# NLAFET/SpLLT

Hardware: AMD Instinct MI355X
Metric: factorize GFLOP/s (fp64) (higher is better)
Workload: dtype f64; 1 GPU; nd24k_like; stand_in_for=SuiteSparse ND/nd24k, n=72324, nnz_lower=10970712, nb=256, nnz_L=190279977, nnodes=684, ordering=user/geometric-nd, parallelism=1 GPU, level-batched stream DAG (chain / bulk / far streams, zone pipeline)

## Files before the change

spllt_amd/csrc/kernels.hip:

```cpp
#include <hip/hip_runtime.h>

#include <cstdint>
#include <cstdlib>
#include <tuple>
#include <type_traits>

#include "kernels.hpp"

#ifndef UPD128_BK
#define UPD128_BK 16
#endif
#ifndef UPD128_WM
#define UPD128_WM 4
#define UPD128_WN 2
#endif

#ifndef UPD64_OCC
#define UPD64_OCC 0
#endif

#if defined(SCATTER_EXPERIMENT) && SCATTER_EXPERIMENT == 1
#define SCATTER_ADD(p, v) (*(p) += (v))
#elif defined(SCATTER_EXPERIMENT) && SCATTER_EXPERIMENT == 2
#define SCATTER_ADD(p, v) (*(p) = (v))
// ... 202 lines not shown
          if (failcol == (1 << 30)) failcol = j;
          djj = 1.0;
        }
        double y, d;
        rsqrt_sqrt(djj, y, d);
        const double sc = row[j] * (y * y);
        wx[j] = (((lr == j) ? 1.0 : 0.0) - wacc[j]) * y;
        const double z = wx[j] * y;
#pragma unroll
        for (int k = j + 1; k < 16; ++k) {
          row[k] -= sc * tk[k];
          wacc[k] = __builtin_fma(tk[k], z, wacc[k]);
        }
        row[j] = (lr == j) ? d : row[j] * y;
        RI[J * 16 + j] = y;
        asm volatile("" : "+v"(wx[j]));
      }
      if (lane < 16) {
#pragma unroll
        for (int c = 0; c < 16; ++c) {
          T[(J * 16 + lr) * TLD + J * 16 + c] = (c <= lr) ? row[c] : 0.0;
          DI[J][c * DLD + lr] = wx[c];
          X[(J * 16 + c) * TLD + J * 16 + lr] = wx[c];
        }
        if (failcol != (1 << 30) && lane == 0 && !(u.flags & 4)) atomicMin(flag, u.gcol + J * 16 + failcol + 1);
      }
    }
    __syncthreads();
    STAMP(3 + 3 * J);
    {
      const int I = J + 1 + w;
      if (I < nblk) {
        d4 acc = {0.0, 0.0, 0.0, 0.0};
#pragma unroll
        for (int t = 0; t < 4; ++t) {
          const double a = T[(I * 16 + lr) * TLD + J * 16 + 4 * t + lq];
          const double b = DI[J][lr * DLD + 4 * t + lq];
          acc = __builtin_amdgcn_mfma_f64_16x16x4f64(a, b, acc, 0, 0, 0);
        }
        st_c(T, I * 16, J * 16, lane, acc);
      }
    }
    __syncthreads();
    STAMP(4 + 3 * J);
  }
  if (!do_chol && w < nblk) {
    double x[16];
#pragma unroll
    for (int i = 0; i < 16; ++i) {
      double sacc = (i == lr) ? 1.0 : 0.0;
#pragma unroll
      for (int k = 0; k < i; ++k) sacc -= T[(w * 16 + i) * TLD + w * 16 + k] * x[k];
      x[i] = (i >= lr) ? sacc * RI[w * 16 + i] : 0.0;
    }
    if (lane < 16) {
#pragma unroll
      for (int i = 0; i < 16; ++i) {
        DI[w][i * DLD + lr] = x[i];
        X[(w * 16 + i) * TLD + w * 16 + lr] = x[i];
      }
    }
  }
  __syncthreads();
  STAMP(14);
  for (int d = 1; d < nblk; ++d) {
    const int J = w, I = J + d;
    if (I < nblk) {
      d4 S = {0.0, 0.0, 0.0, 0.0};
      for (int K = J; K < I; ++K) {
#pragma unroll
        for (int k = 0; k < 16; k += 4) {
          const double a = T[(I * 16 + lr) * TLD + K * 16 + k + lq];
          const double b = X[(K * 16 + k + lq) * TLD + J * 16 + lr];
          S = __builtin_amdgcn_mfma_f64_16x16x4f64(a, b, S, 0, 0, 0);
        }
      }
      d4 R = {0.0, 0.0, 0.0, 0.0};
#pragma unroll
      for (int t = 0; t < 4; ++t) {
        const double a = -DI[I][lr * DLD + 4 * t + lq];
        R = __builtin_amdgcn_mfma_f64_16x16x4f64(a, S[t], R, 0, 0, 0);
      }
      st_c(X, I * 16, J * 16, lane, R);
    }
    __syncthreads();
  }
  STAMP(15);
  if (tid < 256 && lc < n) {
    const bool st_l = do_chol && !(u.flags & 2), st_i = !(u.flags & 4);
#pragma unroll
    for (int e = 0; e < 16; ++e) {
      const int r = 4 * e + lw;
      if (r < n) {
        if (st_l && lc <= r) A[(int64_t)r * ld + lc] = T[r * TLD + lc];
        if (st_i) D[(int64_t)r * ldd + lc] = X[r * TLD + lc];
      }
    }
  }
  STAMP(16);
  (void)np;
}

template <int B, int E, class F>
__device__ __forceinline__ void static_for(F&& f) {
  if constexpr (B < E) {
    f(std::integral_constant<int, B>{});
    static_for<B + 1, E>(f);
  }
}
template <int K>
__device__ __forceinline__ void fmac_bc(double& acc, double s0, double s1) {
  asm volatile("v_fmac_f64_dpp %0, %1, %2 row_newbcast:%3 row_mask:0xf bank_mask:0xf" : "+v"(acc) : "v"(s0), "v"(s1), "n"(K));
}
template <int K>
__device__ __forceinline__ void fmac_bc_pivot(double& acc, double s0, double s1, double& d) {
  asm volatile("v_fmac_f64_dpp %0, %2, %3 row_newbcast:%4 row_mask:0xf bank_mask:0xf\n\ts_nop 1\n\t"
               "v_mov_b64_dpp %1, %0 row_newbcast:%4 row_mask:0xf bank_mask:0xf"
               : "+v"(acc), "=&v"(d) : "v"(s0), "v"(s1), "n"(K));
}
__device__ __forceinline__ double rcp_newton(double d) {
  double y = __builtin_amdgcn_rcp(d);
  y = __builtin_fma(y, __builtin_fma(-d, y, 1.0), y);
  y = __builtin_fma(y, __builtin_fma(-d, y, 1.0), y);
  return y;
}
__device__ __forceinline__ double a_rcp(double d) {
  double y;
  asm volatile("v_rcp_f64 %0, %1\n\ts_nop 0" : "=v"(y) : "v"(d));
  return y;
}
__device__ __forceinline__ double a_nr_err(double d, double y) {
  double e;
  asm volatile("v_fma_f64 %0, -%1, %2, 1.0" : "=v"(e) : "v"(d), "v"(y));
  return e;
}
__device__ __forceinline__ void a_nr_fix(double& y, double e) {
  asm volatile("v_fma_f64 %0, %0, %1, %0" : "+v"(y) : "v"(e));
}
__device__ __forceinline__ double a_nmul(double a, double b) {
  double o;
  asm volatile("v_mul_f64 %0, %1, -%2" : "=v"(o) : "v"(a), "v"(b));
  return o;
}
__device__ __forceinline__ double a_mul(double a, double b) {
  double o;
  asm volatile("v_mul_f64 %0, %1, %2" : "=v"(o) : "v"(a), "v"(b));
  return o;
}
__device__ __forceinline__ double a_sub(double a, double b) {
  double o;
  asm volatile("v_add_f64 %0, %1, -%2" : "=v"(o) : "v"(a), "v"(b));
  return o;
}
__device__ __forceinline__ int chol16_regs(double (&row)[16], double (&wx)[16], int lr) {
  double wacc[16], delta[16];
#pragma unroll
  for (int c = 0; c < 16; ++c) {
    wacc[c] = 0.0;
    delta[c] = (lr == c) ? 1.0 : 0.0;
  }
  double dn = bcast_row<0>(row[0]);
  double dmine = dn;
  double y = rcp_newton(dn);
  STAMP2(true, 21);
  static_for<0, 16>([&](auto jc) {
    constexpr int j = decltype(jc)::value;
    using std::integral_constant;
    const double nsc = a_nmul(row[j], y);
    if constexpr (j + 1 < 16) {
      constexpr int nR = 14 - j, nF = 29 - 2 * j;
      double wxj = 0.0, z = 0.0;
      auto fill = [&](auto lo, auto hi) {
        static_for<decltype(lo)::value, decltype(hi)::value>([&](auto ic) {
          constexpr int i = decltype(ic)::value;
          if constexpr (i < nR) {
            fmac_bc<j + 2 + i>(row[j + 2 + i], row[j], nsc);
          } else {
            if constexpr (i == nR) {
              wxj = a_sub(delta[j], wacc[j]);
              z = a_mul(wxj, y);
            }
            fmac_bc<j + 1 + i - nR>(wacc[j + 1 + i - nR], row[j], z);
          }
        });
      };
      constexpr int b0 = nF * 30 / 100, b1 = nF * 44 / 100, b2 = nF * 58 / 100, b3 = nF * 72 / 100;
      fmac_bc_pivot<j + 1>(row[j + 1], row[j], nsc, dn);
      double yn = a_rcp(dn);
      fill(integral_constant<int, 0>{}, integral_constant<int, b0>{});
      double e = a_nr_err(dn, yn);
      fill(integral_constant<int, b0>{}, integral_constant<int, b1>{});
      a_nr_fix(yn, e);
      fill(integral_constant<int, b1>{}, integral_constant<int, b2>{});
      e = a_nr_err(dn, yn);
      fill(integral_constant<int, b2>{}, integral_constant<int, b3>{});
      a_nr_fix(yn, e);
      fill(integral_constant<int, b3>{}, integral_constant<int, nF>{});
      dmine = (lr == j + 1) ? dn : dmine;
      wx[j] = wxj;
      y = yn;
    } else {
      wx[j] = delta[j] - wacc[j];
    }
  });
  STAMP2(true, 22);
  double ys, rs;
  rsqrt_sqrt(dmine, ys, rs);
  static_for<0, 16>([&](auto cc) {
    constexpr int c = decltype(cc)::value;
    const double sc = bcast_row<c>(ys);
    row[c] *= sc;
    wx[c] *= sc;
    asm volatile("" : "+v"(row[c]), "+v"(wx[c]));
  });
  (void)rs;
  STAMP2(true, 23);
  const unsigned long long bad = __ballot(!(dmine > 0.0)) & 0xffffull;
  return bad ? __builtin_ctzll(bad) : (1 << 30);
}

__device__ __forceinline__ void potrf64_v2(PotrfShared& sh, double* __restrict__ A, int ld, int n,
                                           double* __restrict__ D, int ldd, int gcol, int flags,
                                           int* __restrict__ flag) {
  double (&T)[64 * TLD] = sh.T;
  double (&X)[64 * TLD] = sh.X;
  const int tid = threadIdx.x;
  const int lane = tid & 63, w = tid >> 6, lq = lane >> 4, lr = lane & 15;
  const int nblk = (n + 15) >> 4;
  const bool st_l = !(flags & 2), st_i = !(flags & 4), x_lower = (flags & 8) != 0;
  STAMP(0);
  const int lw = tid >> 6, lc = tid & 63;
  if (flags & 16) {
    if (tid < 256) {
#pragma unroll
      for (int e = 0; e < 16; ++e) X[(4 * e + lw) * TLD + lc] = 0.0;
    }
  } else
  if (tid < 256) {
    double v[16];
#pragma unroll
    for (int e = 0; e < 16; ++e) {
      const int r = 4 * e + lw;
      const int cmax = min(n - 1, r | 15);
      v[e] = A[(int64_t)(r < n ? r : n - 1) * ld + (lc < cmax ? lc : cmax)];
    }
#pragma unroll
    for (int e = 0; e < 16; ++e) X[(4 * e + lw) * TLD + lc] = 0.0;
#pragma unroll
    for (int e = 0; e < 16; ++e) {
      const int r = 4 * e + lw;
      T[r * TLD + lc] = (r < n && lc <= r) ? v[e] : ((r == lc) ? 1.0 : 0.0);
    }
  }
  __syncthreads();
  STAMP(1);
  auto store_rows8 = [&](double* __restrict__ dst, int ldst, const double* M, int row0, int col0) {
    const int g = row0 + (lane >> 3), c = col0 + 2 * (lane & 7);
    const int cend = min(g, n - 1);
    if (g >= n || c > cend) return;
    const double v0 = M[g * TLD + c], v1 = M[g * TLD + c + 1];
    double* q = dst + (int64_t)g * ldst + c;
    if (c + 1 <= cend) {
      typedef double d2 __attribute__((ext_vector_type(2), aligned(8)));
      *reinterpret_cast<d2*>(q) = (d2){v0, v1};
    } else {
      q[0] = v0;
    }
  };
  auto upd_block = [&](int I, int Jp, int S) {
    d4 acc = ld_c(T, I * 16, Jp * 16, lane);
    double a[4], b[4];
#pragma unroll
    for (int t = 0; t < 4; ++t) {
      a[t] = -T[(I * 16 + lr) * TLD + S * 16 + 4 * t + lq];
      b[t] = T[(Jp * 16 + lr) * TLD + S * 16 + 4 * t + lq];
    }
#pragma unroll
    for (int t = 0; t < 4; ++t) acc = __builtin_amdgcn_mfma_f64_16x16x4f64(a[t], b[t], acc, 0, 0, 0);
    st_c(T, I * 16, Jp * 16, lane, acc);
  };
  d4 Xpre = {0.0, 0.0, 0.0, 0.0};
  auto shadow = [&](int S, int ws, int ns, bool stores) {
    const int K = ws;
    if (K < S) {
      d4 R = {0.0, 0.0, 0.0, 0.0};
#pragma unroll
      for (int tt = 0; tt < 4; ++tt) {
        const double a = -X[(S * 16 + lr) * TLD + S * 16 + 4 * tt + lq];
        R = __builtin_amdgcn_mfma_f64_16x16x4f64(a, Xpre[tt], R, 0, 0, 0);
      }
      st_c(X, S * 16, K * 16, lane, R);
      if (st_i && x_lower) {
#pragma unroll
        for (int r = 0; r < 4; ++r) {
          const int g = S * 16 + lq + 4 * r;
          if (g < n) D[(int64_t)g * ldd + K * 16 + lr] = R[r];
        }
      }
    }
    int t = 0;
    for (int Jp = S + 1; Jp < nblk; ++Jp)
      for (int I = Jp; I < nblk; ++I) {
        if (I == S + 1 && Jp == S + 1) continue;
        if (t++ % ns == ws) upd_block(I, Jp, S);
      }
    if (S + 1 < nblk && K <= S) {
      Xpre = (d4){0.0, 0.0, 0.0, 0.0};
      for (int M = K; M <= S; ++M) {
#pragma unroll
        for (int k = 0; k < 16; k += 4) {
          const double a = T[((S + 1) * 16 + lr) * TLD + M * 16 + k + lq];
          const double b = X[(M * 16 + k + lq) * TLD + K * 16 + lr];
          Xpre = __builtin_amdgcn_mfma_f64_16x16x4f64(a, b, Xpre, 0, 0, 0);
        }
      }
    }
    if (!stores) return;
    const int ngrp = (64 - S * 16) / 8;
    for (int gi = ws; gi < ngrp; gi += ns)
      if (st_l) store_rows8(A, ld, T, S * 16 + gi * 8, S * 16);
    if (st_i && x_lower)
      for (int gi = ws; gi < 2; gi += ns) store_rows8(D, ldd, X, S * 16 + gi * 8, S * 16);
  };
  for (int J = 0; J < nblk; ++J) {
    if (w == 0) {
      if (J > 0) upd_block(J, J, J - 1);
      double row[16], wx[16];
      STAMP2(true, 20);
#pragma unroll
      for (int c = 0; c < 16; ++c) row[c] = T[(J * 16 + lr) * TLD + J * 16 + c];
      const int failcol = chol16_regs(row, wx, lr);
      STAMP2(true, 24);
      if (lq == 0) {
        double* dst = &T[(J * 16 + lr) * TLD + J * 16];
#pragma unroll
        for (int c = 0; c < 16; ++c) dst[c] = row[c];
        if (failcol != (1 << 30) && lane == 0 && st_i) atomicMin(flag, gcol + J * 16 + failcol + 1);
      } else if (lq == 1) {
        double* dst = &X[(J * 16) * TLD + J * 16 + lr];
#pragma unroll
        for (int c = 0; c < 16; ++c) dst[c * TLD] = wx[c];
      }
      STAMP2(true, 25);
    } else if (w < 4 && J > 0) {
      shadow(J - 1, w - 1, 3, true);
    }
    __syncthreads();
    STAMP(2 + 2 * J);
    if (w < 4 && J + 1 + w < nblk) {
      const int I = J + 1 + w;
      d4 acc = {0.0, 0.0, 0.0, 0.0};
#pragma unroll
      for (int t = 0; t < 4; ++t) {
        const double a = T[(I * 16 + lr) * TLD + J * 16 + 4 * t + lq];
        const double b = X[(J * 16 + lr) * TLD + J * 16 + 4 * t + lq];
        acc = __builtin_amdgcn_mfma_f64_16x16x4f64(a, b, acc, 0, 0, 0);
      }
      st_c(T, I * 16, J * 16, lane, acc);
    }
    __syncthreads();
    STAMP(3 + 2 * J);
  }
  if (w > 0 && w < 4) {
    const int S = nblk - 1, K = w - 1;
    if (K < S) shadow(S, K, 3, false);
  } else if (w == 0) {
    const int S = nblk - 1;
    if (st_l) { store_rows8(A, ld, T, S * 16, S * 16); store_rows8(A, ld, T, S * 16 + 8, S * 16); }
    if (st_i && x_lower) { store_rows8(D, ldd, X, S * 16, S * 16); store_rows8(D, ldd, X, S * 16 + 8, S * 16); }
  }
  STAMP(10);
  if (st_i && !x_lower) {
    __syncthreads();
    if (tid < 256)
      for (int r = lw; r < n; r += 4)
        if (lc < n) D[(int64_t)r * ldd + lc] = X[r * TLD + lc];
  }
  STAMP(11);
}

__device__ __forceinline__ void potrf64(PotrfShared& sh, double* __restrict__ A, int ld, int n,
                                        double* __restrict__ D, int ldd, int gcol, int flags,
                                        int* __restrict__ flag) {
#ifndef POTRF_V1
  if (!(flags & 1)) {
    potrf64_v2(sh, A, ld, n, D, ldd, gcol, flags, flag);
    return;
  }
#endif
  potrf64_body(sh, A, ld, n, D, ldd, gcol, flags, flag);
}

__global__ __launch_bounds__(256) void k_potrf_panel(const PotrfUnit* __restrict__ units,
                                                     double* __restrict__ L,
                                                     double* __restrict__ dinv,
                                                     int* __restrict__ flag, const PotrfUnit u0) {
  __shared__ PotrfShared sh;
  __builtin_amdgcn_s_setprio(3);
  const PotrfUnit u = blockIdx.x == 0 ? u0 : units[blockIdx.x];
  potrf64(sh, L + u.off, u.ld, u.n, dinv + u.dinv_off, u.n, u.gcol, u.flags, flag);
}

__global__ __launch_bounds__(256) void k_chain_potrf(const ChainUnit* __restrict__ units,
                                                     double* __restrict__ L,
                                                     double* __restrict__ dinv,
                                                     int* __restrict__ flag, const ChainUnit u0) {
  __shared__ PotrfShared sh;
  __builtin_amdgcn_s_setprio(3);
  const ChainUnit u = blockIdx.x == 0 ? u0 : units[blockIdx.x];
  const int cq = u.c0 - u.cs;
  potrf64(sh, L + u.off + (int64_t)u.c0 * u.ld + u.c0, u.ld, u.pn, dinv + u.winv_off + cq, u.ce - u.cs,
          u.gcol, 8, flag);
}

constexpr int kPanelThreads = 512;

__device__ __forceinline__ void stage_block(double* __restrict__ dst, const double* __restrict__ src,
                                            int64_t ld, int nrow, int ncol, int tid) {
  const int r = tid >> 3, cl = tid & 7;
  const double* row = src + (int64_t)(r < nrow ? r : nrow - 1) * ld;
  double v[8];
#pragma unroll
  for (int e = 0; e < 8; ++e) v[e] = row[cl + 8 * e < ncol ? cl + 8 * e : ncol - 1];
#pragma unroll
  for (int e = 0; e < 8; ++e) dst[r * TLD + cl + 8 * e] = (r < nrow && cl + 8 * e < ncol) ? v[e] : 0.0;
}

__device__ __forceinline__ void mma_64(const double* __restrict__ a, const double* __restrict__ b, int s,
                                       int jb0, int lane, d4& acc0, d4& acc1) {
  const int lq = lane >> 4, lr = lane & 15;
  double av[16], b0[16], b1[16];
#pragma unroll
  for (int kt = 0; kt < 16; ++kt) {
    av[kt] = a[(s * 16 + lr) * TLD + 4 * kt + lq];
    b0[kt] = b[(jb0 * 16 + lr) * TLD + 4 * kt + lq];
    b1[kt] = b[((jb0 + 1) * 16 + lr) * TLD + 4 * kt + lq];
  }
#pragma unroll
  for (int kt = 0; kt < 16; ++kt) {
    acc0 = __builtin_amdgcn_mfma_f64_16x16x4f64(av[kt], b0[kt], acc0, 0, 0, 0);
    acc1 = __builtin_amdgcn_mfma_f64_16x16x4f64(av[kt], b1[kt], acc1, 0, 0, 0);
  }
}

__device__ __forceinline__ void mma_64_lean(const double* __restrict__ a, const double* __restrict__ b, int s,
                                            int jb0, int lane, d4& acc0, d4& acc1) {
  const int lq = lane >> 4, lr = lane & 15;
#pragma unroll
  for (int hf = 0; hf < 2; ++hf) {
    double av[8], b0[8], b1[8];
#pragma unroll
    for (int kt = 0; kt < 8; ++kt) {
      av[kt] = a[(s * 16 + lr) * TLD + 4 * (8 * hf + kt) + lq];
      b0[kt] = b[(jb0 * 16 + lr) * TLD + 4 * (8 * hf + kt) + lq];
      b1[kt] = b[((jb0 + 1) * 16 + lr) * TLD + 4 * (8 * hf + kt) + lq];
    }
#pragma unroll
    for (int kt = 0; kt < 8; ++kt) {
      acc0 = __builtin_amdgcn_mfma_f64_16x16x4f64(av[kt], b0[kt], acc0, 0, 0, 0);
      acc1 = __builtin_amdgcn_mfma_f64_16x16x4f64(av[kt], b1[kt], acc1, 0, 0, 0);
    }
    asm volatile("" ::: "memory");
  }
}

__device__ __forceinline__ void mma_64x4(const double* __restrict__ a, const double* __restrict__ b, int s,
                                         int lane, d4 (&acc)[4]) {
#pragma unroll
  for (int q = 0; q < 4; ++q) acc[q] = (d4){0.0, 0.0, 0.0, 0.0};
  mma_64(a, b, s, 0, lane, acc[0], acc[1]);
  mma_64(a, b, s, 2, lane, acc[2], acc[3]);
}

__device__ __forceinline__ bool last_reader(int* __restrict__ counter, int readers, int* __restrict__ slot) {
  if (threadIdx.x == 0) {
    __threadfence();
    const int old = atomicAdd(counter, 1);
    const bool last = old == readers - 1;
    if (last) atomicExch(counter, 0);
    *slot = last ? 1 : 0;
  }
  __syncthreads();
  const bool last = *slot != 0;
  __syncthreads();
  return last;
}

__global__ __launch_bounds__(kPanelThreads) void k_panel(const UpdTile* __restrict__ tiles,
                                                         const PanelUnit* __restrict__ units,
                                                         double* __restrict__ L,
                                                         double* __restrict__ dinv,
                                                         int* __restrict__ counters,
                                                         int* __restrict__ flag) {
  extern __shared__ __attribute__((aligned(16))) double panel_smem[];
  __shared__ int vote;
  PotrfShared& sh = *reinterpret_cast<PotrfShared*>(panel_smem);
  double* Ui = sh.T;
  double* Ud = panel_smem + sizeof(PotrfShared) / sizeof(double);
  double* S = Ud + 64 * TLD;
  __builtin_amdgcn_s_setprio(3);
  const UpdTile tl = tiles[blockIdx.x];
  const PanelUnit u = units[tl.unit];
  const int tid = threadIdx.x, lane = tid & 63, wave = tid >> 6, lq = lane >> 4, lr = lane & 15;
  const int ld = u.ld, c0 = u.c0, pn = u.pn;
  double* A = L + u.off;
  const bool first = tl.ti == 0;
  double* Dg = A + (int64_t)c0 * ld + c0;
  const bool factored = (u.pad_ & 1) != 0;
  if (factored) {
    const double* W = dinv + u.dinv_off;
    for (int e = tid; e < 64 * 64; e += kPanelThreads) {
      const int r = e >> 6, c = e & 63;
      sh.X[r * TLD + c] = (r < pn && c <= r) ? W[(int64_t)r * pn + c] : 0.0;
    }
  } else {
    potrf64(sh, Dg, ld, pn, dinv + u.dinv_off, pn, u.gcol, first ? (2 | 8) : 6, flag);
  }
  __syncthreads();
  if (!factored && last_reader(counters + 2 * tl.unit, u.ntile, &vote)) {
    const int lc = tid & 63;
#pragma unroll
    for (int e = 0; e < 8; ++e) {
      const int r = 8 * e + (tid >> 6);
      if (r < pn && lc <= r) Dg[(int64_t)r * ld + lc] = sh.T[r * TLD + lc];
    }
    __syncthreads();
  }
  const int r1 = c0 + pn;
  const int r0 = r1 + 64 * (int)tl.ti;
  const int nr = min(64, u.nrow - r0);
  if (nr <= 0) return;
  const int pn2 = u.next_pn;
  const int s = wave >> 1, jb0 = (wave & 1) * 2;
  stage_block(S, A + (int64_t)r0 * ld + c0, ld, nr, pn, tid);
  __syncthreads();
  bool store_pivot = pn2 > 0 && first && last_reader(counters + 2 * tl.unit + 1, u.ntile, &vote);
  {
    d4 a0 = {0.0, 0.0, 0.0, 0.0}, a1 = {0.0, 0.0, 0.0, 0.0};
    mma_64(S, sh.X, s, jb0, lane, a0, a1);
#pragma unroll
    for (int r = 0; r < 4; ++r) {
      const int i = s * 16 + lq + 4 * r;
#pragma unroll
      for (int h = 0; h < 2; ++h) {
        const int j = (jb0 + h) * 16 + lr;
        const double v = (j < pn) ? (h ? a1[r] : a0[r]) : 0.0;
        Ui[i * TLD + j] = v;
        const bool mine = !first || i >= pn2 || store_pivot;
        if (mine && i < nr && j < pn) A[(int64_t)(r0 + i) * ld + c0 + j] = v;
      }
    }
  }
  if (pn2 <= 0) return;
  __syncthreads();
  const double* Xd = Ui;
  if (!first) {
    stage_block(S, A + (int64_t)r1 * ld + c0, ld, pn2, pn, tid);
    __syncthreads();
    store_pivot = last_reader(counters + 2 * tl.unit + 1, u.ntile, &vote);
    d4 a0 = {0.0, 0.0, 0.0, 0.0}, a1 = {0.0, 0.0, 0.0, 0.0};
// ... 1377 lines not shown
  const double* A = L + u.off + (int64_t)r0 * w;
  const int* idx = rlist + u.idx_off;
  if (!BWD) {
    for (int k = tid; k < w; k += 256) {
      const int gi = u.gcol0 + k;
#pragma unroll
      for (int q = 0; q < NR; ++q) xb[q * kXS + k] = y[q * ldy + gi];
    }
    __syncthreads();
    const int sub = tid & 15, rr = tid >> 4;
    double acc[4][NR];
#pragma unroll
    for (int r = 0; r < 4; ++r)
      dot16<NR, kXS>(A + (int64_t)min(rr + 16 * r, nr - 1) * w, xb, w, sub, acc[r]);
#pragma unroll
    for (int r = 0; r < 4; ++r) {
      const int row = rr + 16 * r;
      const int gi = idx[r0 + min(row, nr - 1)];
#pragma unroll
      for (int q = 0; q < NR; ++q) {
        const double sacc = sum16(acc[r][q]);
        if (sub == 0 && row < nr) unsafeAtomicAdd(y + q * ldy + gi, -sacc);
      }
    }
  } else {
    for (int r = tid; r < nr; r += 256) {
      const int gi = idx[r0 + r];
#pragma unroll
      for (int q = 0; q < NR; ++q) xb[q * kXS + r] = y[q * ldy + gi];
    }
    __syncthreads();
    for (int k = tid; k < w; k += 256) {
      double sa[NR];
#pragma unroll
      for (int q = 0; q < NR; ++q) sa[q] = 0.0;
      for (int q0 = 0; q0 < nr; q0 += 8) {
        double v[8];
#pragma unroll
        for (int e = 0; e < 8; ++e) v[e] = A[(int64_t)min(q0 + e, nr - 1) * w + k];
#pragma unroll
        for (int e = 0; e < 8; ++e) {
          const double a = q0 + e < nr ? v[e] : 0.0;
#pragma unroll
          for (int q = 0; q < NR; ++q) sa[q] = __builtin_fma(a, xb[q * kXS + min(q0 + e, nr - 1)], sa[q]);
        }
      }
      const int gi = u.gcol0 + k;
#pragma unroll
      for (int q = 0; q < NR; ++q) unsafeAtomicAdd(y + q * ldy + gi, -sa[q]);
    }
  }
}

template <int NR>
static void launch_solve_nr(hipStream_t st, int kind, const int* list, const UpdTile* tiles,
                            int64_t first, int64_t count, const SolveUnit* units, const double* L,
                            const double* dinv, const int* rlist, double* y, int64_t ldy, bool four,
                            const SolveUnit* one) {
  const dim3 g((unsigned)count), b(256);
  const SolveUnit u0 = one ? *one : SolveUnit{};
  const int single = one ? 1 : 0;
  switch (kind) {
    case SV_DIAG_FWD:
      if (four)
        hipLaunchKernelGGL((k_solve_diag4<false, NR>), g, b, 0, st, list + first, units, L, dinv, rlist, y, ldy, u0, single);
      else
        hipLaunchKernelGGL((k_solve_diag<false, NR>), g, b, 0, st, list + first, units, L, dinv, rlist, y, ldy, u0, single);
      break;
    case SV_DIAG_BWD:
      if (four)
        hipLaunchKernelGGL((k_solve_diag4<true, NR>), g, b, 0, st, list + first, units, L, dinv, rlist, y, ldy, u0, single);
      else
        hipLaunchKernelGGL((k_solve_diag<true, NR>), g, b, 0, st, list + first, units, L, dinv, rlist, y, ldy, u0, single);
      break;
    case SV_STRIP_FWD:
      hipLaunchKernelGGL((k_solve_strip<false, NR>), g, b, 0, st, tiles + first, units, L, rlist, y, ldy, u0, single);
      break;
    default:
      hipLaunchKernelGGL((k_solve_strip<true, NR>), g, b, 0, st, tiles + first, units, L, rlist, y, ldy, u0, single);
      break;
  }
}

void launch_solve(hipStream_t st, int kind, const int* list, const UpdTile* tiles, int64_t first,
                  int64_t count, const SolveUnit* units, const double* L, const double* dinv,
                  const int* rlist, double* y, int nr, int64_t ldy, bool four, const SolveUnit* one) {
  if (count <= 0) return;
  if (nr >= 4)
    launch_solve_nr<4>(st, kind, list, tiles, first, count, units, L, dinv, rlist, y, ldy, four, one);
  else if (nr >= 2)
    launch_solve_nr<2>(st, kind, list, tiles, first, count, units, L, dinv, rlist, y, ldy, four, one);
  else
    launch_solve_nr<1>(st, kind, list, tiles, first, count, units, L, dinv, rlist, y, ldy, four, one);
}

void launch_expand_buffer(hipStream_t st, double* a, int blkn, const int* row_list, int rls,
                          const int* col_list, int cls, int ndiag, const double* buffer) {
  if (rls <= 0 || cls <= 0) return;
  int blocks = (rls + 3) / 4;
  if (blocks > 2048) blocks = 2048;
  hipLaunchKernelGGL(k_expand_buffer, dim3(blocks), dim3(256), 0, st, a, blkn, row_list, rls,
                     col_list, cls, ndiag, buffer);
}

__global__ __launch_bounds__(256) void k_init_arena(double* __restrict__ L, int64_t arena,
                                                    const double* __restrict__ val,
                                                    const int64_t* __restrict__ cptr,
                                                    const unsigned short* __restrict__ loc,
                                                    const int* __restrict__ src) {
  __shared__ __attribute__((aligned(16))) double img[kInitChunk];
  const int tid = threadIdx.x;
  const int64_t c = blockIdx.x;
  const int64_t e0 = cptr[c], e1 = cptr[c + 1];
  for (int e = tid; e < kInitChunk; e += 256) img[e] = 0.0;
  __syncthreads();
  for (int64_t e = e0 + tid; e < e1; e += 256) img[loc[e]] = val[src[e]];
  __syncthreads();
  const int64_t base = c * kInitChunk;
  const int64_t n = arena - base < kInitChunk ? arena - base : kInitChunk;
  typedef double d2v __attribute__((ext_vector_type(2)));
  if (n == kInitChunk) {
    d2v* out = reinterpret_cast<d2v*>(L + base);
    const d2v* in = reinterpret_cast<const d2v*>(img);
    for (int e = tid; e < kInitChunk / 2; e += 256) out[e] = in[e];
  } else {
    for (int64_t e = tid; e < n; e += 256) L[base + e] = img[e];
  }
}

void launch_init_arena(const LaunchSink& st, double* L, int64_t arena, const double* val, const int64_t* cptr,
                       const unsigned short* loc, const int* src) {
  if (arena <= 0) return;
  const int64_t chunks = (arena + kInitChunk - 1) / kInitChunk;
  emit(st, k_init_arena, dim3((unsigned)chunks), dim3(256), 0, L, arena, val, cptr, loc, src);
}

void launch_scatter_val(const LaunchSink& st, double* L, const double* val, const int64_t* dst,
                        const int64_t* src, int64_t n) {
  if (n <= 0) return;
  int64_t blocks = (n + 255) / 256;
  if (blocks > 2048) blocks = 2048;
  emit(st, k_scatter_val, dim3((unsigned)blocks), dim3(256), 0, L, val, dst, src, n);
}

void launch_potrf(hipStream_t st, const PotrfUnit* units, int64_t count, double* L, double* dinv,
                  int* flag, const PotrfUnit& unit0) {
  if (count <= 0) return;
  hipLaunchKernelGGL(k_potrf_panel, dim3((unsigned)count), dim3(256), 0, st, units, L, dinv, flag, unit0);
}

void launch_chain_panel(const LaunchSink& st, const ChainUnit* units, int64_t count, double* L, double* dinv,
                        int* flag, const ChainUnit& unit0) {
  if (count <= 0) return;
  emit(st, k_chain_potrf, dim3((unsigned)count), dim3(256), 0, units, L, dinv, flag, unit0);
}

void launch_chain_block(const LaunchSink& st, const ChainUnit* units, int64_t count, double* L, double* dinv,
                        int* flag, int pw, const ChainUnit& unit0) {
  if (count <= 0) return;
  const unsigned lds = (unsigned)(sizeof(PotrfShared) + sizeof(double) * 2 * 64 * TLD);
  thread_local int attr_dev = -1;
  int dev = 0;
  (void)hipGetDevice(&dev);
  if (dev != attr_dev) {
    (void)hipFuncSetAttribute((const void*)k_chain_block, hipFuncAttributeMaxDynamicSharedMemorySize, (int)lds);
    attr_dev = dev;
  }
  emit(st, k_chain_block, dim3((unsigned)count), dim3(kPanelThreads), lds, units, L, dinv, flag, pw, unit0);
}

void launch_subtree(const LaunchSink& st, const SubTask* tasks, int64_t count, const SubNode* nodes,
                    const UpdUnit* units, const int* relpos, const int* rlist, double* L, double* dinv, double* gen,
                    int* flag) {
  if (count <= 0) return;
  emit(st, k_subtree, dim3((unsigned)count), dim3(kSubThreads), 0, tasks, nodes, units, relpos, rlist, L, dinv, gen, flag);
}

void launch_trsm_rows(const LaunchSink& st, const UpdTile* tiles, int64_t count, const UpdUnit* units, double* L,
                      const double* dinv, int pw, int prio) {
  if (count <= 0) return;
  const unsigned lds = (unsigned)(sizeof(double) * 2 * 64 * TLD);
  thread_local int attr_dev = -1;
  int dev = 0;
  (void)hipGetDevice(&dev);
  if (dev != attr_dev) {
    (void)hipFuncSetAttribute((const void*)k_trsm_rows, hipFuncAttributeMaxDynamicSharedMemorySize, (int)lds);
    attr_dev = dev;
  }
  emit(st, k_trsm_rows, dim3((unsigned)count), dim3(256), lds, tiles, units, L, dinv, pw, prio);
}

void launch_panel(const LaunchSink& st, const UpdTile* tiles, int64_t count, const PanelUnit* units, double* L,
                  double* dinv, int* counters, int* flag) {
  if (count <= 0) return;
  const unsigned lds = (unsigned)(sizeof(PotrfShared) + sizeof(double) * 2 * 64 * TLD);
  thread_local int attr_dev = -1;
  int dev = 0;
  (void)hipGetDevice(&dev);
  if (dev != attr_dev) {
    (void)hipFuncSetAttribute((const void*)k_panel, hipFuncAttributeMaxDynamicSharedMemorySize, (int)lds);
    attr_dev = dev;
  }
  emit(st, k_panel, dim3((unsigned)count), dim3(kPanelThreads), lds, tiles, units, L, dinv, counters, flag);
}

__global__ __launch_bounds__(256) void k_gather(const GatherTile* __restrict__ tiles,
                                                const GatherItem* __restrict__ items,
                                                double* __restrict__ L,
                                                const double* __restrict__ scratch,
                                                const int* __restrict__ relpos,
                                                const int* __restrict__ rlist) {
  __shared__ double acc[64 * 65];
  const GatherTile t = tiles[blockIdx.x];
  const int tid = threadIdx.x;
  for (int e = tid; e < 64 * 65; e += 256) acc[e] = 0.0;
  __syncthreads();
  for (int it = 0; it < t.count; ++it) {
    const GatherItem g = items[t.first + it];
    const int ni = g.i1 - g.i0, nj = g.j1 - g.j0;
    const double* buf = scratch + g.buf_off;
    for (int e = tid; e < ni * nj; e += 256) {
      const int i = g.i0 + e / nj, j = g.j0 + e % nj;
      if (g.lower && g.diag_shift + i < j) continue;
      const int r = relpos[g.relrow_off + i] - t.drow_base - t.row0;
      const int c = rlist[g.gcol_off + j] - t.dcol_base - t.col0;
      acc[r * 65 + c] += buf[(int64_t)i * g.ld + j];
    }
    __syncthreads();
  }
  double* D = L + t.d_off + (int64_t)t.row0 * t.d_ld + t.col0;
  for (int e = tid; e < t.rows * t.cols; e += 256) {
    const int r = e / t.cols, c = e % t.cols;
    const double a = acc[r * 65 + c];
    if (a != 0.0) D[(int64_t)r * t.d_ld + c] -= a;
  }
}

void launch_gather(const LaunchSink& st, const GatherTile* tiles, int64_t count, const GatherItem* items,
                   double* L, const double* scratch, const int* relpos, const int* rlist) {
  if (count <= 0) return;
  emit(st, k_gather, dim3((unsigned)count), dim3(256), 0, tiles, items, L, scratch, relpos, rlist);
}

__global__ void k_flag_pack(const int* __restrict__ flag, double* __restrict__ slot) {
  *slot = (*flag != 0x7fffffff) ? 1.0 : 0.0;
}
__global__ void k_flag_unpack(const double* __restrict__ slot, int* __restrict__ flag) {
  if (*slot > 0.5 && *flag == 0x7fffffff) *flag = 0x7ffffffe;
}
__global__ __launch_bounds__(256) void k_mask(double* __restrict__ y, const double* __restrict__ keep, int n,
                                              int nrhs, int64_t ldy) {
  const int i = blockIdx.x * 256 + threadIdx.x;
  if (i >= n) return;
  const double k = keep[i];
  for (int q = 0; q < nrhs; ++q) y[q * ldy + i] *= k;
}
void launch_mask(hipStream_t st, double* y, const double* keep, int n, int nrhs, int64_t ldy) {
  if (n <= 0 || nrhs <= 0) return;
  hipLaunchKernelGGL(k_mask, dim3((unsigned)((n + 255) / 256)), dim3(256), 0, st, y, keep, n, nrhs, ldy);
}
void launch_flag_pack(hipStream_t st, const int* flag, double* slot) {
  hipLaunchKernelGGL(k_flag_pack, dim3(1), dim3(1), 0, st, flag, slot);
}
void launch_flag_unpack(hipStream_t st, const double* slot, int* flag) {
  hipLaunchKernelGGL(k_flag_unpack, dim3(1), dim3(1), 0, st, slot, flag);
}

__global__ __launch_bounds__(256) void k_poison_lds(int* sink) {
  extern __shared__ __attribute__((aligned(16))) double poison_smem[];
  const double snan = __longlong_as_double(0x7FF4DEADBEEF0001LL);
  for (int i = threadIdx.x; i < 160 * 1024 / 8; i += 256) poison_smem[i] = snan;
  __syncthreads();
  if (sink && poison_smem[threadIdx.x] == 0.0) *sink = 1;
}

void launch_poison_lds(hipStream_t st) {
  thread_local int attr_dev = -1;
  int dev = 0;
  (void)hipGetDevice(&dev);
  if (dev != attr_dev) {
    (void)hipFuncSetAttribute((const void*)k_poison_lds, hipFuncAttributeMaxDynamicSharedMemorySize,
                              160 * 1024);
    attr_dev = dev;
  }
  hipLaunchKernelGGL(k_poison_lds, dim3(1024), dim3(256), 160 * 1024, st, (int*)nullptr);
}

void launch_update(const LaunchSink& st, int tile, const UpdTile* tiles, int64_t count,
                   const UpdUnit* units, const int64_t* bc_off, const int* bc_w, double* L,
                   const int* relpos, const int* rlist, const double* dinv, int prio,
                   int lds_pad, bool allow_dma, bool latency) {
  if (count <= 0) return;
  static const int lat_bk = [] { const char* e = std::getenv("SPLLT_LAT_BK"); return e ? std::atoi(e) : 0; }();
  if (latency && lat_bk == 64 && (tile == 64 || tile == 32)) {
    thread_local int attr_dev3 = -1;
    int dev3 = 0;
    (void)hipGetDevice(&dev3);
    if (dev3 != attr_dev3) {
      (void)hipFuncSetAttribute((const void*)k_update<64, 64, 2, 2>, hipFuncAttributeMaxDynamicSharedMemorySize, 150 * 1024);
      (void)hipFuncSetAttribute((const void*)k_update<32, 64, 2, 2>, hipFuncAttributeMaxDynamicSharedMemorySize, 150 * 1024);
      attr_dev3 = dev3;
    }
    const unsigned lds = (unsigned)(sizeof(double) * 2 * UPD_STAGES * tile * (64 + UPD_LDK_PAD));
    if (tile == 64)
      emit(st, k_update<64, 64, 2, 2>, dim3((unsigned)count), dim3(256), lds, tiles, units, bc_off, bc_w, L, relpos,
           rlist, dinv, prio);
    else
// ... 65 lines not shown
```

Before: 32220 GFLOP/s.

## Streamline chol16 register math, split potrf64 loop by wave, and tune chain potrf kernel

The 16x16 Cholesky now seeds the inverse accumulator with -1 on the diagonal and negates it, which removes the delta array and saves registers and subtractions. The wave index is made uniform with readfirstlane, and the per-J loop is split into a wave-0 branch and a branch for the other waves so the branch is hoisted out of the loop. k_chain_potrf gets launch_bounds(256,4) and dynamic LDS with an attribute set at launch. Together these aim to cut register pressure and branching in the small panel factorization and raise occupancy, though the split loops must still hit identical __syncthreads counts.

```diff
diff --git a/spllt_amd/csrc/kernels.hip b/spllt_amd/csrc/kernels.hip
--- a/spllt_amd/csrc/kernels.hip
+++ b/spllt_amd/csrc/kernels.hip
@@ -378,13 +378,15 @@
   asm volatile("v_add_f64 %0, %1, -%2" : "=v"(o) : "v"(a), "v"(b));
   return o;
 }
+__device__ __forceinline__ double a_neg0(double a) {
+  double o;
+  asm volatile("v_add_f64 %0, 0, -%1" : "=v"(o) : "v"(a));
+  return o;
+}
 __device__ __forceinline__ int chol16_regs(double (&row)[16], double (&wx)[16], int lr) {
-  double wacc[16], delta[16];
-#pragma unroll
-  for (int c = 0; c < 16; ++c) {
-    wacc[c] = 0.0;
-    delta[c] = (lr == c) ? 1.0 : 0.0;
-  }
+  double wacc[16];
+#pragma unroll
+  for (int c = 0; c < 16; ++c) wacc[c] = (lr == c) ? -1.0 : 0.0;
   double dn = bcast_row<0>(row[0]);
   double dmine = dn;
   double y = rcp_newton(dn);
@@ -403,7 +405,7 @@
             fmac_bc<j + 2 + i>(row[j + 2 + i], row[j], nsc);
           } else {
             if constexpr (i == nR) {
-              wxj = a_sub(delta[j], wacc[j]);
+              wxj = a_neg0(wacc[j]);
               z = a_mul(wxj, y);
             }
             fmac_bc<j + 1 + i - nR>(wacc[j + 1 + i - nR], row[j], z);
@@ -426,7 +428,7 @@
       wx[j] = wxj;
       y = yn;
     } else {
-      wx[j] = delta[j] - wacc[j];
+      wx[j] = a_neg0(wacc[j]);
     }
   });
   STAMP2(true, 22);
@@ -451,11 +453,11 @@
   double (&T)[64 * TLD] = sh.T;
   double (&X)[64 * TLD] = sh.X;
   const int tid = threadIdx.x;
-  const int lane = tid & 63, w = tid >> 6, lq = lane >> 4, lr = lane & 15;
+  const int lane = tid & 63, w = __builtin_amdgcn_readfirstlane(tid >> 6), lq = lane >> 4, lr = lane & 15;
   const int nblk = (n + 15) >> 4;
   const bool st_l = !(flags & 2), st_i = !(flags & 4), x_lower = (flags & 8) != 0;
   STAMP(0);
-  const int lw = tid >> 6, lc = tid & 63;
+  const int lw = w, lc = tid & 63;
   if (flags & 16) {
     if (tid < 256) {
 #pragma unroll
@@ -548,8 +550,21 @@
     if (st_i && x_lower)
       for (int gi = ws; gi < 2; gi += ns) store_rows8(D, ldd, X, S * 16 + gi * 8, S * 16);
   };
-  for (int J = 0; J < nblk; ++J) {
-    if (w == 0) {
+  auto solve_below = [&](int J) {
+    if (w < 4 && J + 1 + w < nblk) {
+      const int I = J + 1 + w;
+      d4 acc = {0.0, 0.0, 0.0, 0.0};
+#pragma unroll
+      for (int t = 0; t < 4; ++t) {
+        const double a = T[(I * 16 + lr) * TLD + J * 16 + 4 * t + lq];
+        const double b = X[(J * 16 + lr) * TLD + J * 16 + 4 * t + lq];
+        acc = __builtin_amdgcn_mfma_f64_16x16x4f64(a, b, acc, 0, 0, 0);
+      }
+      st_c(T, I * 16, J * 16, lane, acc);
+    }
+  };
+  if (w == 0) {
+    for (int J = 0; J < nblk; ++J) {
       if (J > 0) upd_block(J, J, J - 1);
       double row[16], wx[16];
       STAMP2(true, 20);
@@ -568,32 +583,26 @@
         for (int c = 0; c < 16; ++c) dst[c * TLD] = wx[c];
       }
       STAMP2(true, 25);
-    } else if (w < 4 && J > 0) {
-      shadow(J - 1, w - 1, 3, true);
-    }
-    __syncthreads();
-    STAMP(2 + 2 * J);
-    if (w < 4 && J + 1 + w < nblk) {
-      const int I = J + 1 + w;
-      d4 acc = {0.0, 0.0, 0.0, 0.0};
-#pragma unroll
-      for (int t = 0; t < 4; ++t) {
-        const double a = T[(I * 16 + lr) * TLD + J * 16 + 4 * t + lq];
-        const double b = X[(J * 16 + lr) * TLD + J * 16 + 4 * t + lq];
-        acc = __builtin_amdgcn_mfma_f64_16x16x4f64(a, b, acc, 0, 0, 0);
-      }
-      st_c(T, I * 16, J * 16, lane, acc);
-    }
-    __syncthreads();
-    STAMP(3 + 2 * J);
-  }
-  if (w > 0 && w < 4) {
-    const int S = nblk - 1, K = w - 1;
-    if (K < S) shadow(S, K, 3, false);
-  } else if (w == 0) {
+      __syncthreads();
+      STAMP(2 + 2 * J);
+      solve_below(J);
+      __syncthreads();
+      STAMP(3 + 2 * J);
+    }
     const int S = nblk - 1;
     if (st_l) { store_rows8(A, ld, T, S * 16, S * 16); store_rows8(A, ld, T, S * 16 + 8, S * 16); }
     if (st_i && x_lower) { store_rows8(D, ldd, X, S * 16, S * 16); store_rows8(D, ldd, X, S * 16 + 8, S * 16); }
+  } else {
+    for (int J = 0; J < nblk; ++J) {
+      if (w < 4 && J > 0) shadow(J - 1, w - 1, 3, true);
+      __syncthreads();
+      solve_below(J);
+      __syncthreads();
+    }
+    if (w < 4) {
+      const int S = nblk - 1, K = w - 1;
+      if (K < S) shadow(S, K, 3, false);
+    }
   }
   STAMP(10);
   if (st_i && !x_lower) {
@@ -627,11 +636,12 @@
   potrf64(sh, L + u.off, u.ld, u.n, dinv + u.dinv_off, u.n, u.gcol, u.flags, flag);
 }
 
-__global__ __launch_bounds__(256) void k_chain_potrf(const ChainUnit* __restrict__ units,
-                                                     double* __restrict__ L,
-                                                     double* __restrict__ dinv,
-                                                     int* __restrict__ flag, const ChainUnit u0) {
-  __shared__ PotrfShared sh;
+__global__ __launch_bounds__(256, 4) void k_chain_potrf(const ChainUnit* __restrict__ units,
+                                                        double* __restrict__ L,
+                                                        double* __restrict__ dinv,
+                                                        int* __restrict__ flag, const ChainUnit u0) {
+  extern __shared__ __attribute__((aligned(16))) double chain_smem[];
+  PotrfShared& sh = *reinterpret_cast<PotrfShared*>(chain_smem);
   __builtin_amdgcn_s_setprio(3);
   const ChainUnit u = blockIdx.x == 0 ? u0 : units[blockIdx.x];
   const int cq = u.c0 - u.cs;
@@ -2315,7 +2325,16 @@
 void launch_chain_panel(const LaunchSink& st, const ChainUnit* units, int64_t count, double* L, double* dinv,
                         int* flag, const ChainUnit& unit0) {
   if (count <= 0) return;
-  emit(st, k_chain_potrf, dim3((unsigned)count), dim3(256), 0, units, L, dinv, flag, unit0);
+  static_assert(sizeof(PotrfShared) <= 80 * 1024, "k_chain_potrf: LDS budget (scripts/check_kernel_budget.py)");
+  const unsigned lds = (unsigned)sizeof(PotrfShared);
+  thread_local int attr_dev = -1;
+  int dev = 0;
+  (void)hipGetDevice(&dev);
+  if (dev != attr_dev) {
+    (void)hipFuncSetAttribute((const void*)k_chain_potrf, hipFuncAttributeMaxDynamicSharedMemorySize, (int)lds);
+    attr_dev = dev;
+  }
+  emit(st, k_chain_potrf, dim3((unsigned)count), dim3(256), lds, units, L, dinv, flag, unit0);
 }
 
 void launch_chain_block(const LaunchSink& st, const ChainUnit* units, int64_t count, double* L, double* dinv,
```

Result: faster. 33000 GFLOP/s, median of 6 (+2.4%).
